# jdhuang-csm/bayes-drt

Hardware: AMD Instinct MI355X
Metric: HMC log-posterior+grad evals/sec (81 freq x 161 tau-basis) (higher is better)
Workload: dtype f64

## Files before the change

### bayes_drt_amd/csrc/bdrt_tile_s1.h

```cpp
#pragma once
#include "bdrt_device.h"
#include <type_traits>

namespace bdrt {

static __device__ long long *g_tile_trace = nullptr;

__device__ __forceinline__ int swz(int row, int col) { return row * NC + (col ^ (row & 15)); }

template <int LPC>
__device__ __forceinline__ double hsum(double x)
{
    x = sum32(x);
    if (LPC == 64) x += __shfl_xor(x, 32);
    return x;
}

__device__ __forceinline__ void wave_sync()
{
    __builtin_amdgcn_fence(__ATOMIC_RELEASE, "wavefront");
    __builtin_amdgcn_wave_barrier();
    __builtin_amdgcn_fence(__ATOMIC_ACQUIRE, "wavefront");
}

// ... 17 lines not shown
#pragma unroll
    for (int e = 0; e < 2; ++e) {
        bX[e] = Bs + kq * NC + (col ^ (8 * e + kq));
        bY[e] = Bs + (kq + 4) * NC + (col ^ (8 * e + kq + 4));
    }
    auto load = [&](dv2 (&buf)[GPF]) {
        gp2 p = base + ((size_t)(wave + l_ti * NWV) * pairs + (size_t)l_ch * GPF) * 64;
#pragma unroll
        for (int i = 0; i < GPF; ++i) buf[i] = p[(size_t)i * 64];
        if (++l_ch == nchunk) { l_ch = 0; ++l_ti; }
    };
    auto step = [&](const dv2 (&cur)[GPF], dv2 (&nxt)[GPF], bool prefetch) {
        const int p0 = c_ch * GPF;
        const bool odd = p0 & 1;
        const double *x0 = (odd ? bX[1] : bX[0]) + p0 * (8 * NC), *x1 = (odd ? bX[0] : bX[1]) + p0 * (8 * NC);
        const double *y0 = (odd ? bY[1] : bY[0]) + p0 * (8 * NC), *y1 = (odd ? bY[0] : bY[1]) + p0 * (8 * NC);
        double bx[GPF], by[GPF];
#pragma unroll
        for (int i = 0; i < GPF; ++i) {
            bx[i] = ((i & 1) ? x1 : x0)[i * (8 * NC)];
            by[i] = ((i & 1) ? y1 : y0)[i * (8 * NC)];
        }
        __builtin_amdgcn_sched_barrier(0);
        acc0 = mfma_f64(cur[0].x, bx[0], acc0);
        acc1 = mfma_f64(cur[0].y, by[0], acc1);
        __builtin_amdgcn_sched_barrier(0);
        if (prefetch) load(nxt);
        __builtin_amdgcn_sched_barrier(0);
#pragma unroll
        for (int i = 1; i < GPF; ++i) {
            acc0 = mfma_f64(cur[i].x, bx[i], acc0);
            acc1 = mfma_f64(cur[i].y, by[i], acc1);
        }
        __builtin_amdgcn_sched_barrier(0);
        if (++c_ch == nchunk) {
            const int t = wave + c_ti * NWV;
#pragma unroll
            for (int rr = 0; rr < 4; ++rr) { const int row = 16 * t + kq + 4 * rr; Os[swz(row, col)] = acc0[rr] + acc1[rr]; }
            acc0 = d4{0.0, 0.0, 0.0, 0.0}; acc1 = d4{0.0, 0.0, 0.0, 0.0};
            c_ch = 0; ++c_ti;
        }
    };
    dv2 a[GPF], b[GPF];
    if (items > 0) load(a);
    for (int it = 0; it < items; it += 2) {
        step(a, b, it + 1 < items);
        if (it + 1 < items) step(b, a, it + 2 < items);
    }
    if (rem > 0) {
        for (int ti = 0; ti < nt; ++ti) {
            const int t = wave + ti * NWV;
            d4 r0a = {0.0, 0.0, 0.0, 0.0}, r1a = {0.0, 0.0, 0.0, 0.0};
            for (int p = nchunk * GPF; p < pairs; ++p) {
                const dv2 v = base[((size_t)t * pairs + p) * 64];
                const int r0 = 8 * p + kq, r1 = r0 + 4;
                r0a = mfma_f64(v.x, Bs[swz(r0, col)], r0a);
                r1a = mfma_f64(v.y, Bs[swz(r1, col)], r1a);
            }
#pragma unroll
            for (int rr = 0; rr < 4; ++rr) {
                const int row = 16 * t + kq + 4 * rr;
                const double prev = nchunk > 0 ? Os[swz(row, col)] : 0.0;
                Os[swz(row, col)] = prev + r0a[rr] + r1a[rr];
            }
        }
    }
}

constexpr int RW = 32 * UK + 2 * MAXBW;
constexpr int NTAP = 2 * MAXBW + 1;
constexpr int WIN = UK + NTAP - 1;

__host__ __device__ inline int s1_ku(int K) { return K <= 64 ? 2 : (K <= 96 ? 3 : (K <= 128 ? 4 : 6)); }
__host__ __device__ inline int s1_nj(int D) { return D <= 32 * 4 ? 4 : (D <= 32 * 6 ? 6 : (D <= 32 * 7 ? 7 : (D <= 32 * 11 ? 11 : 16))); }
__host__ __device__ inline int s1_zrows(const DevProblem &P) { return P.toepA == 2 ? P.zrows : 16 * P.blk[0].tilesA; }
template <int TA> __device__ __forceinline__ constexpr int toep_pad() { return TA == 2 ? 16 : 8; }
template <int TA> __device__ __forceinline__ int toep_im_row(int nf) { return TA == 2 ? (nf + 3) & ~3 : nf; }

__device__ __forceinline__ const double *s1_toep_table(const DevProblem &P, const double *smem)
{
    return smem + (size_t)NC * (P.XR + s1_zrows(P)) + (size_t)2 * NC * RW;
}

#ifndef BDRT_TOEP_STAMP
#define BDRT_TOEP_STAMP(slot)
#endif
template <bool FWD>
__device__ __forceinline__ void toep_gemm(int nf, int K, int tlen, const double *Tt, const double *Bs, double *Os, int wave, int lane)
{
    typedef const __attribute__((address_space(3))) double *lds_cptr;
    const int i = lane & 15, kq = lane >> 4, col = i;
    wave = __builtin_amdgcn_readfirstlane(wave);
    constexpr int TPP = 5;
    const int r4 = nf & 3;
    const int T = FWD ? 2 * TPP : (K >> 4);
    const int base = T & ~7, R = T - base;
    const int nqt = FWD ? (K >> 4) : 2 * TPP;
    const bool halves = R > 0 && R <= 4 && nqt % 10 == 0;
    const int npiece = base + (halves ? 2 * R : R);
    if (wave >= npiece) return;
    BDRT_TOEP_STAMP(0);

    const lds_cptr aL = (lds_cptr)(Tt + (FWD ? i - kq - 76 : kq - i));
    lds_cptr bL0 = (lds_cptr)(Bs + swz(kq, col)), bL1 = (lds_cptr)(Bs + swz(4 + kq, col)), bL2 = (lds_cptr)(Bs + swz(8 + kq, col)),
             bL3 = (lds_cptr)(Bs + swz(12 + kq, col));
    const int dI0 = FWD ? 0 : swz(nf + kq, col) - swz(kq, col), dI1 = FWD ? 0 : swz(nf + 4 + kq, col) - swz(4 + kq, col),
              dI2 = FWD ? 0 : swz(nf + 8 + kq, col) - swz(8 + kq, col), dI3 = FWD ? 0 : swz(nf + 12 + kq, col) - swz(12 + kq, col);
    const int mpart = kq >= r4 ? 1 : 0, mn = nf - r4 + kq - mpart * r4;
    const lds_cptr mL = (lds_cptr)(Tt + mpart * tlen + 8 + mn - i + (K - 1));
    double Bm = 0.0;
    if (!FWD && r4) Bm = Bs[swz(kq < 2 * r4 ? mpart * nf + mn : 2 * nf + kq, col)];

    int t = 0, half = -1, orow = 0, nblk = 0, nrem = 0, aoff = 0, boff = 0;
    bool mixed = false;
    lds_cptr a, b0, b1, b2, b3;
    double A0[4], B0[4], A1[4], B1[4], A2[4], B2[4], Am = 0.0;
    d4 acc0 = {0.0, 0.0, 0.0, 0.0}, acc1 = {0.0, 0.0, 0.0, 0.0};

    auto describe = [&](int sidx) {
        t = sidx; half = -1;
        if (sidx >= base && halves) { t = base + ((sidx - base) >> 1); half = (sidx - base) & 1; }
        if (FWD) {
            const int part = t >= TPP ? 1 : 0, n0 = 16 * (t - part * TPP);
            orow = part * nf + n0;
            const int nch = (K + 3) >> 2, nq = nch >> 2;
            const int q0 = half == 1 ? nq / 2 : 0, q1 = half == 0 ? nq / 2 : nq;
            nblk = (q1 - q0) / 5; nrem = half == 0 ? 0 : nch & 3;
            aoff = part * tlen + 8 + n0 + (K - 1) - 16 * q0;
            boff = 16 * NC * q0;
            mixed = false;
        } else {
            orow = 16 * t;
            nblk = half < 0 ? 2 : 1; nrem = 0;
            aoff = 8 - 16 * t + (K - 1); boff = 0;
            mixed = r4 != 0 && half != 0;
        }
    };
    auto set_ptrs = [&](int blk) {
        if (FWD) {
            a = aL + (aoff - 80 * blk);
            const int o = boff + 80 * NC * blk;
            b0 = bL0 + o; b1 = bL1 + o; b2 = bL2 + o; b3 = bL3 + o;
        } else {
            const bool im = half == 1 || blk == 1;
            a = aL + (aoff + (im ? tlen : 0));
            b0 = bL0 + (im ? dI0 : 0); b1 = bL1 + (im ? dI1 : 0); b2 = bL2 + (im ? dI2 : 0); b3 = bL3 + (im ? dI3 : 0);
        }
    };
    auto ld = [&](double (&A)[4], double (&B)[4], auto Rr) {
        constexpr int r = decltype(Rr)::value;
#pragma unroll
        for (int j = 0; j < 4; ++j) A[j] = FWD ? a[76 - 16 * r - 4 * j] : a[16 * r + 4 * j];
        B[0] = b0[16 * NC * r]; B[1] = b1[16 * NC * r]; B[2] = b2[16 * NC * r]; B[3] = b3[16 * NC * r];
    };
    typedef std::integral_constant<int, 0> R0;
    typedef std::integral_constant<int, 1> R1;
    typedef std::integral_constant<int, 2> R2;
    typedef std::integral_constant<int, 3> R3;
    typedef std::integral_constant<int, 4> R4;
    auto mm = [&](const double (&A)[4], const double (&B)[4], auto &&next) {
        acc0 = mfma_f64(A[0], B[0], acc0);
        __builtin_amdgcn_sched_barrier(0);
        next();
        __builtin_amdgcn_sched_barrier(0);
        acc1 = mfma_f64(A[1], B[1], acc1);
        acc0 = mfma_f64(A[2], B[2], acc0);
        acc1 = mfma_f64(A[3], B[3], acc1);
        __builtin_amdgcn_sched_barrier(0);
    };
    auto block = [&](auto &&after) {
        mm(A2, B2, [&]() { ld(A0, B0, R1()); });
        mm(A0, B0, [&]() { ld(A1, B1, R2()); });
        mm(A1, B1, [&]() { ld(A0, B0, R3()); });
        mm(A0, B0, [&]() { ld(A1, B1, R4()); });
        mm(A1, B1, after);
    };
    auto open = [&](int sidx) {
        describe(sidx);
        set_ptrs(0);
        ld(A2, B2, R0());
        if (!FWD && mixed) Am = mL[-16 * t];
    };

    open(wave);
    BDRT_TOEP_STAMP(1);
    for (int sidx = wave; sidx < npiece; sidx += 8) {
        const bool more = sidx + 8 < npiece;
        const int o_row = orow, o_half = half, o_nrem = nrem;
        const bool o_mixed = mixed;
        const double o_Am = Am;
        const int nb = nblk;
        for (int blk = 0; blk < nb; ++blk) {
            const bool last = blk + 1 == nb;
            block([&]() {
                if (!last) { set_ptrs(blk + 1); ld(A2, B2, R0()); }
                else if (FWD && o_nrem) { set_ptrs(nb); ld(A2, B2, R0()); }
                else if (more) open(sidx + 8);
            });
        }
        if (FWD && o_nrem) {
            double ra[3] = {A2[0], A2[1], A2[2]}, rb[3] = {B2[0], B2[1], B2[2]};
            acc0 = mfma_f64(ra[0], rb[0], acc0);
            if (o_nrem > 1) acc1 = mfma_f64(ra[1], rb[1], acc1);
            if (o_nrem > 2) acc0 = mfma_f64(ra[2], rb[2], acc0);
            __builtin_amdgcn_sched_barrier(0);
            if (more) open(sidx + 8);
        }
        if (!FWD && o_mixed) acc1 = mfma_f64(o_Am, Bm, acc1);
        __builtin_amdgcn_sched_barrier(0);
        BDRT_TOEP_STAMP(2 + 3 * (sidx >> 3));
        const d4 s = acc0 + acc1;
        BDRT_TOEP_STAMP(3 + 3 * (sidx >> 3));
#pragma unroll
        for (int rr = 0; rr < 4; ++rr) {
            double *o = Os + swz(o_row + kq + 4 * rr, col);
            if (o_half < 0) *o = s[rr];
            else __hip_atomic_fetch_add(o, s[rr], __ATOMIC_RELAXED, __HIP_MEMORY_SCOPE_WORKGROUP);
        }
        acc0 = d4{0.0, 0.0, 0.0, 0.0}; acc1 = d4{0.0, 0.0, 0.0, 0.0};
        BDRT_TOEP_STAMP(4 + 3 * (sidx >> 3));
    }
}

template <bool FWD>
__device__ __forceinline__ void toep_zero_split(int nf, int K, double *Os, int tid)
{
    const int TPP = nf >> 4, T = FWD ? 2 * TPP : (K >> 4);
    const int base = T & ~7, R = T - base;
    if (R == 0 || R > 4 || (FWD ? (K >> 4) : 2 * TPP) % 10 != 0) return;
    for (int e = tid; e < R * 256; e += NT) {
        const int t = base + (e >> 8), r = (e >> 4) & 15;
        const int part = (FWD && t >= TPP) ? 1 : 0;
        const int row = FWD ? part * nf + 16 * (t - part * TPP) + r : 16 * t + r;
        Os[row * NC + (e & 15)] = 0.0;
    }
}

struct ToepSched { int base, R, mode, npiece; };
__host__ __device__ inline ToepSched toep_sched(int T, bool can_halve)
{
    ToepSched sc;
    sc.base = T & ~7; sc.R = T - sc.base;
    sc.mode = (sc.R == 0 || !can_halve || sc.R == 7) ? 0 : (sc.R <= 4 ? 1 : 2);
    sc.npiece = sc.base + (sc.mode == 0 ? sc.R : (sc.mode == 1 ? 2 * sc.R : 2 * sc.R - 4));
    return sc;
}
__host__ __device__ inline int toep_gen_tiles(int m) { return (m & 15) <= 2 ? (m >> 4) : ((m + 15) >> 4); }
__host__ __device__ inline int toep_gen_odd(int m) { return (m & 15) <= 2 ? (m & 15) : 0; }

constexpr int TOEP_STEPS = 8;
constexpr int TOEP_STEP_WORDS = 2 * 8 * TOEP_STEPS * 2;
inline int toep_gen_steps(bool fwd, int nf, int K, int tlen, int wave, unsigned *out)
{
    const int PAD = 16;
    const int nfi = (nf + 3) & ~3;
    const int TPP = fwd ? toep_gen_tiles(nf) : 0;
    const int T = fwd ? 2 * TPP : toep_gen_tiles(K);
    const int nch = fwd ? (K + 3) >> 2 : nfi >> 2;
    const int nq = nch >> 2;
    const int qsplit = (nq + 1) >> 1;
    const int lim = fwd ? nf : K;
    if (nq < 2 || nq > 12) return -1;
    const ToepSched sc = toep_sched(T, fwd ? nq >= 4 : true);
    int n = 0;
    bool shared_seen = false;
    auto emit = [&](int part, int n0, int q0, int kind, int shared) {
        const int aoff = fwd ? part * tlen + PAD + n0 + (K - 1) - 16 * q0 : part * tlen + PAD - n0 + (K - 1);
        const int orow = fwd ? part * nfi + n0 : n0;
        int room = lim - n0; room = room > 16 ? 16 : room;
        if (aoff < 0 || aoff > 65535 || q0 > 255 || orow > 4095 || n >= TOEP_STEPS - 1) return -1;
        out[2 * n] = (unsigned)aoff | (unsigned)q0 << 16 | (unsigned)kind << 24 | (unsigned)(fwd ? 0 : part) << 30;
        out[2 * n + 1] = (unsigned)orow | (unsigned)room << 12 | (unsigned)shared << 21 | 1u << 24;
        ++n;
        return 0;
    };
    for (int s = wave; s < sc.npiece; s += 8) {
        int t = s, half = -1;
        if (s >= sc.base) {
            const int j = s - sc.base;
            if (sc.mode == 1) { t = sc.base + (j >> 1); half = j & 1; }
            else if (sc.mode == 2 && j >= 4) { t = sc.base + 4 + ((j - 4) >> 1); half = (j - 4) & 1; }
        }
        if (shared_seen) return -1;
        if (half >= 0) shared_seen = true;
        if (fwd) {
            const int part = t >= TPP ? 1 : 0, n0 = 16 * (t - part * TPP);
            if (emit(part, n0, half == 1 ? qsplit : 0, half + 1, half >= 0 ? 1 : 0)) return -1;
        } else if (half < 0) {
            if (emit(0, 16 * t, 0, 0, 0) || emit(1, 16 * t, 0, 0, 0)) return -1;
        } else if (emit(half, 16 * t, 0, 0, 1)) return -1;
    }
    const int runs = n;
    if (runs == 0) { out[0] = (unsigned)(PAD + K - 1); out[1] = 0; }
    else { out[2 * n] = out[0]; out[2 * n + 1] = out[1] & ~(1u << 24); }
    ++n;
    for (; n < TOEP_STEPS; ++n) { out[2 * n] = out[2 * runs]; out[2 * n + 1] = out[2 * runs + 1]; }
    return runs;
}

template <int I, int N, class F>
__device__ __forceinline__ void toep_static_for(F &&f)
{
// ... 89 lines not shown
    if (!((c1 >> 24) & 1u)) return;
    prefetch(c0);
    auto body = [&](auto Lc) {
        constexpr int L = decltype(Lc)::value;
        int st = 1;
        if (FWD) {
            while (((c1 >> 24) & 1u) && ((c0 >> 24) & 3u) == 0) {
                const unsigned n0w = __builtin_amdgcn_readlane(w0v, st), n1w = __builtin_amdgcn_readlane(w1v, st);
                ++st;
                run(Lc, Tr(), n0w, nr);
                store(c1);
                c0 = n0w; c1 = n1w;
            }
            if ((c1 >> 24) & 1u) {
                const unsigned n0w = __builtin_amdgcn_readlane(w0v, st);
                if (((c0 >> 24) & 3u) == 1) run(std::integral_constant<int, (L + 1) / 2 >= 2 ? (L + 1) / 2 : 2>(), Tr(), n0w, 0);
                else run(std::integral_constant<int, L / 2 >= 2 ? L / 2 : 2>(), Tr(), n0w, nr);
                store(c1);
            }
        } else {
            while (((c1 >> 24) & 1u) && !((c1 >> 21) & 1u)) {
                const unsigned m0w = __builtin_amdgcn_readlane(w0v, st);
                const unsigned n0w = __builtin_amdgcn_readlane(w0v, st + 1), n1w = __builtin_amdgcn_readlane(w1v, st + 1);
                st += 2;
                run(Lc, Tr(), m0w, nr);
                run(Lc, Fa(), n0w, nr);
                store(c1);
                c0 = n0w; c1 = n1w;
            }
            if ((c1 >> 24) & 1u) {
                const unsigned n0w = __builtin_amdgcn_readlane(w0v, st);
                run(Lc, Tr(), n0w, nr);
                store(c1);
            }
        }
    };
    switch (nq) {
    case 2: body(std::integral_constant<int, 2>()); break;
    case 3: body(std::integral_constant<int, 3>()); break;
    case 4: body(std::integral_constant<int, 4>()); break;
    case 5: body(std::integral_constant<int, 5>()); break;
    case 6: body(std::integral_constant<int, 6>()); break;
    case 7: body(std::integral_constant<int, 7>()); break;
    case 8: body(std::integral_constant<int, 8>()); break;
    case 9: if constexpr (FWD) body(std::integral_constant<int, 9>()); break;
    case 10: if constexpr (FWD) body(std::integral_constant<int, 10>()); break;
    case 11: if constexpr (FWD) body(std::integral_constant<int, 11>()); break;
    case 12: if constexpr (FWD) body(std::integral_constant<int, 12>()); break;
    default: break;
    }
}

template <bool FWD>
__device__ __forceinline__ void toep_zero_split_gen(int nf, int K, double *Os, int tid)
{
    const int nfi = (nf + 3) & ~3;
    const int TPP = FWD ? toep_gen_tiles(nf) : 0;
    const int T = FWD ? 2 * TPP : toep_gen_tiles(K);
    const ToepSched sc = toep_sched(T, FWD ? (((K + 3) >> 2) >> 2) >= 4 : true);
    if (sc.mode == 0) return;
    const int first = sc.mode == 1 ? sc.base : sc.base + 4, cnt = sc.mode == 1 ? sc.R : sc.R - 4;
    for (int e = tid; e < cnt * 256; e += NT) {
        const int t = first + (e >> 8), r = (e >> 4) & 15;
        const int part = (FWD && t >= TPP) ? 1 : 0;
        const int n = FWD ? 16 * (t - part * TPP) + r : 16 * t + r;
        if (n < (FWD ? nf : K)) Os[(FWD ? part * nfi + n : n) * NC + (e & 15)] = 0.0;
    }
}

__device__ __forceinline__ void s1_toep_init(const DevProblem &P, double *smem)
{
    const DevBlock &B = P.blk[0];
    double *Tt = const_cast<double *>(s1_toep_table(P, smem));
    double *Zh = smem + (size_t)P.XR * NC;
    const int glen = P.nf + B.K - 1, tlen = P.tlen, pad = P.toepA == 2 ? 16 : 8;
    for (int e = threadIdx.x; e < 2 * tlen; e += NT) {
        const int part = e >= tlen ? 1 : 0, j = e - part * tlen - pad;
        Tt[e] = (j >= 0 && j < glen) ? B.tg[(size_t)part * glen + j] : 0.0;
    }
    if (P.toepA == 2) {
        unsigned *st = (unsigned *)(Tt + 2 * tlen);
        for (int e = threadIdx.x; e < TOEP_STEP_WORDS; e += NT) st[e] = P.tsteps[e];
    }
    for (int e = (P.toepA == 2 ? 0 : 2 * P.nf * NC) + threadIdx.x; e < s1_zrows(P) * NC; e += NT) Zh[e] = 0.0;
    __syncthreads();
}

__device__ __forceinline__ double *s1_grad_row(const DevProblem &P, double *smem, int c);


__host__ __device__ inline size_t s1_lds_doubles(const DevProblem &P)
{
    return (size_t)NC * (P.XR + s1_zrows(P)) + (size_t)2 * NC * RW + (P.toepA ? (size_t)2 * P.tlen : 0) + (P.toepA == 2 ? (size_t)TOEP_STEP_WORDS / 2 : 0);
}

struct NoHook { __device__ __forceinline__ void operator()() const {} };

template <bool LDSIO, int LPC = 32, class Hook = NoHook, class Hook1 = NoHook, int TA = 0, int KU = 6>
__device__ inline void logp_grad_tile_s1(const DevProblem &P, const TileIO &io, double *smem, Hook before_backward = Hook(),
                                         Hook1 after_x_ready = Hook1())
{
    int tid = threadIdx.x;
    __asm__ volatile("" : "+v"(tid));
    constexpr int UKV = 32 * KU / LPC, UNV = 128 / LPC, WINV = UKV + NTAP - 1, NWV = 16 * LPC / 64;
    constexpr int GPFV = LPC == 32 ? 7 : 3;
    const int lane = tid & 63, wave = tid >> 6;
    const int c = tid / LPC;
    const int l32 = tid % LPC, hb = lane & (64 - LPC);
    const DevBlock &B = P.blk[0];
    const int nf = P.nf, N2 = 2 * nf, K = B.K, KP = 8 * B.kpairs;
    const int omode = LDSIO ? 0 : P.outlier_mode;
    const int dbg = P.dbg;
    const bool valid = c < io.nvalid;
    const int cc = valid ? c : 0;
    const double jac = io.jacobian ? 1.0 : 0.0;

    double *Xs = smem;
    double *Zh = Xs + (size_t)P.XR * NC;
    double *xrow = Zh + (size_t)(TA == 2 ? P.zrows : 16 * B.tilesA) * NC + (size_t)c * (2 * RW);
    double *wrow = xrow + RW;

    const double *th = io.theta + (long)cc * io.t_sc;
    typedef const __attribute__((address_space(3))) double *lds_cptr;
    auto TH = [&](int j) -> double { return LDSIO ? ((lds_cptr)th)[j] : th[(long)j * io.t_sj]; };
    double *gr = (io.grad && valid) ? io.grad + (long)cc * io.g_sc : nullptr;
    auto GW = [&](int j, double v) { if (!LDSIO && gr) gr[(long)j * io.g_sj] = v; };
    double gsc = 0.0;
    double *pr = (!LDSIO && io.params && valid) ? io.params + (size_t)cc * P.D : nullptr;
    auto PW = [&](int j, double v) { if (!LDSIO && pr) pr[j] = v; };

    long long tprev = (io.prof && tid == 0) ? clock64() : 0;
    long long *trc = g_tile_trace ? g_tile_trace + ((size_t)blockIdx.x * NWV + wave) * 16 : nullptr;
#define BDRT_S1_TRACE(slot) do { if (trc && (lane == 0)) trc[slot] = clock64(); } while (0)
    BDRT_S1_TRACE(0);
#define BDRT_S1_PROF(slot) do { if (io.prof && tid == 0) { const long long t_ = clock64(); io.prof[slot] += t_ - tprev; tprev = t_; } } while (0)
    long long twe = io.prof ? clock64() : 0;
#define BDRT_S1_BARRIER(slot, wslot) do { if (io.prof) { const long long tb_ = clock64(); __syncthreads(); const long long te_ = clock64(); \
        if (lane == 0) { atomicAdd((unsigned long long *)&io.prof[slot], (unsigned long long)(te_ - tb_)); \
                         if (wslot) atomicAdd((unsigned long long *)&io.prof[wslot], (unsigned long long)(tb_ - twe)); } \
        twe = te_; } else __syncthreads(); } while (0)

    double sraw = 0.0, st = 0.0;
    {
        int j = -1;
        if (l32 < 2) j = l32;
        else if (l32 < 6) j = P.o_err + (l32 - 2);
        else if (l32 < 9) j = B.o_d + (l32 - 6);
        if (j >= 0) { st = TH(j); sraw = lean_exp(st); PW(j, sraw); }
    }
    double lp = 0.0;
    int lp_lane = -1;
    double x_[UKV];
    {
        double tx_[UKV], tu_[UKV];
#pragma unroll
        for (int u = 0; u < UKV; ++u) {
            const int k = l32 + LPC * u, kk = k < K ? k : 0;
            tx_[u] = TH(B.o_x + kk);
            tu_[u] = TH(B.o_ups + kk);
        }
#pragma unroll
        for (int u = 0; u < UKV; ++u) {
            const bool in = l32 + LPC * u < K;
            tx_[u] = in ? tx_[u] : 0.0;
            tu_[u] = in ? tu_[u] : 0.0;
        }
        double ex_[UKV];
#pragma unroll
        for (int u = 0; u < UKV; ++u) ex_[u] = lean_exp(tx_[u]);
#pragma unroll
        for (int u = 0; u < UKV; ++u) {
            const int k = l32 + LPC * u;
            double xr = 0.0;
            if (k < K) {
                xr = B.is_pos ? ex_[u] : tx_[u];
                if (B.is_pos) lp += jac * tx_[u];
                PW(B.o_x + k, xr);
            }
            x_[u] = xr;
            if (k < KP) Xs[swz(k, c)] = xr;
            xrow[MAXBW + k] = xr;
            wrow[MAXBW + k] = tu_[u];
        }
        if (l32 < MAXBW) {
            xrow[l32] = 0.0; xrow[MAXBW + LPC * UKV + l32] = 0.0;
            wrow[l32] = 0.0; wrow[MAXBW + LPC * UKV + l32] = 0.0;
        }
    }
    static_assert(!TA || LPC == 32, "the Toeplitz-A GEMMs are written for 512 threads");
    const double *Tt = TA ? s1_toep_table(P, smem) : nullptr;
    const int tlen = TA ? P.tlen : 0;
    constexpr int TPAD = toep_pad<TA>();
    const int nfi = toep_im_row<TA>(nf);
    if (TA) {
        const int r16 = TA == 2 ? toep_gen_odd(nf) : (nf & 15), n0 = nf - r16;
        for (int j = 0; j < r16; ++j) {
            double sr = 0.0, si = 0.0;
#pragma unroll
            for (int u = 0; u < UKV; ++u) {
                const int idx = max(TPAD + n0 + j + (K - 1) - (l32 + LPC * u), 0);
                sr = fma(Tt[idx], x_[u], sr); si = fma(Tt[tlen + idx], x_[u], si);
            }
            sr = hsum<LPC>(sr); si = hsum<LPC>(si);
            if (l32 == 0) { Zh[swz(n0 + j, c)] = sr; Zh[swz(nfi + n0 + j, c)] = si; }
        }
        if (TA == 2) toep_zero_split_gen<true>(nf, K, Zh, tid); else toep_zero_split<true>(nf, K, Zh, tid);
    }
    const double d0 = __shfl(sraw, hb | 6), d1 = __shfl(sraw, hb | 7), d2 = __shfl(sraw, hb | 8);
    const double israw5 = 5.0 * lean_rcp(sraw);
    if (l32 < 6) lp += -0.5 * sraw * sraw + jac * st;
    else if (l32 < 9) lp += -6.0 * st - israw5 + jac * st;
#ifndef BDRT_SPEC_EARLY
#define BDRT_SPEC_EARLY 0
#endif
#ifndef BDRT_EARLY_P2
#define BDRT_EARLY_P2 1
#endif
#ifndef BDRT_P2_OPAQUE_K
#define BDRT_P2_OPAQUE_K 1
#endif
    constexpr bool EARLY_P2 = BDRT_EARLY_P2 != 0;
    double zre_[UNV], zim_[UNV], wn_[UNV];
    auto load_spectrum = [&]() {
        const int sp = io.spec ? io.spec[cc] : 0;
        const double *Zm = P.Z + (size_t)sp * N2;
#pragma unroll
        for (int v = 0; v < UNV; ++v) {
            const int n = l32 + LPC * v, nn = n < nf ? n : 0;
            zre_[v] = Zm[nn]; zim_[v] = Zm[nf + nn]; wn_[v] = P.w[nn];
        }
    };
#pragma unroll 1
    for (int step = 0; step < 2; ++step) {
    if (EARLY_P2 ? step == 1 : step == 0) {
        BDRT_S1_TRACE(1);
        BDRT_S1_BARRIER(25, 29);
        after_x_ready();
        if constexpr (BDRT_SPEC_EARLY) load_spectrum();
        BDRT_S1_TRACE(2);
        BDRT_S1_PROF(1);
        BDRT_S1_TRACE(3);
        if (!(dbg & 1)) {
            if (TA == 2) toep_gemm_gen<true>(nf, K, tlen, Tt, Xs, Zh, wave, lane);
            else if (TA) toep_gemm<true>(nf, K, tlen, Tt, Xs, Zh, wave, lane);
            else gemm_sw<NWV, GPFV>(B.Af, B.tilesA, B.kpairs, Xs, Zh, wave, lane);
        }
        continue;
    }

    BDRT_S1_TRACE(4);
    if (!(dbg & 4)) {
        const int kb = UKV * l32;
        double xw[WINV], tuc[UKV];
#pragma unroll
        for (int j = 0; j < WINV; ++j) xw[j] = xrow[kb + j];
#pragma unroll
        for (int u = 0; u < UKV; ++u) tuc[u] = wrow[MAXBW + kb + u];
        wave_sync();
        double v0_[UKV], v1_[UKV], v2_[UKV];
#pragma unroll
        for (int u = 0; u < UKV; ++u) { v0_[u] = 0.0; v1_[u] = 0.0; v2_[u] = 0.0; }
        double tn0 = B.T[0][0], tn1 = B.T[1][0], tn2 = B.T[2][0];
#pragma unroll
        for (int d = 0; d < NTAP; ++d) {
            const double t0 = tn0, t1 = tn1, t2 = tn2;
            if (d + 1 < NTAP) { tn0 = B.T[0][d + 1]; tn1 = B.T[1][d + 1]; tn2 = B.T[2][d + 1]; }
            __asm__ volatile("" ::: "memory");
#pragma unroll
            for (int u = 0; u < UKV; ++u) { v0_[u] = fma(t0, xw[u + d], v0_[u]); v1_[u] = fma(t1, xw[u + d], v1_[u]); v2_[u] = fma(t2, xw[u + d], v2_[u]); }
        }
        double ue[UKV + 4], ie[UKV + 2];
#pragma unroll
        for (int u = 0; u < UKV; ++u) { ue[u + 2] = 0.15 * lean_exp(tuc[u]); ie[u + 1] = lean_rcp(ue[u + 2]); }
        {
            const int lo = hb | ((l32 + LPC - 1) & (LPC - 1)), hi = hb | ((l32 + 1) & (LPC - 1));
            ue[0] = __shfl(ue[UKV], lo); ue[1] = __shfl(ue[UKV + 1], lo);
            ue[UKV + 2] = __shfl(ue[2], hi); ue[UKV + 3] = __shfl(ue[3], hi);
            ie[0] = __shfl(ie[UKV], lo); ie[UKV + 1] = __shfl(ie[1], hi);
        }
        BDRT_S1_PROF(5);
        double sv0 = 0, sv1 = 0, sv2 = 0;
        double w0_[UKV], w1_[UKV], w2_[UKV], gup[UKV];
#pragma unroll
        for (int u = 0; u < UKV; ++u) {
            int k = kb + u;
#if BDRT_P2_OPAQUE_K
            __asm__ volatile("" : "+v"(k));
#endif
            w0_[u] = 0.0; w1_[u] = 0.0; w2_[u] = 0.0; gup[u] = 0.0;
            if (k < K) {
                const double um2 = ue[u], um1 = ue[u + 1], uu = ue[u + 2], up1 = ue[u + 3], up2 = ue[u + 4];
                const double t = tuc[u];
                const double iu = ie[u + 1], iu2 = iu * iu;
                const double v0 = v0_[u], v1 = v1_[u], v2 = v2_[u];
                const double q2 = d0 * v0 * v0 + d1 * v1 * v1 + d2 * v2 * v2;
                const double ir = 0.15 * iu;
                lp += -(t + LOG_015) - 0.5 * q2 * iu2 - (P.ups_alpha + 1.0) * t - P.ups_beta * ir + jac * t;
                sv0 += v0 * v0 * iu2; sv1 += v1 * v1 * iu2; sv2 += v2 * v2 * iu2;
                double gu = -iu + q2 * iu2 * iu;
                if (k >= 1 && k + 1 < K) {
                    const double du = 0.5 * (uu - 0.5 * (um1 + up1)) * iu;
                    lp += -0.5 * du * du;
                    gu += -du * 0.25 * (um1 + up1) * iu2;
                }
                if (k >= 2) {
                    const double i0 = ie[u];
                    const double du = 0.5 * (um1 - 0.5 * (um2 + uu)) * i0;
                    gu += du * 0.25 * i0;
                }
                if (k + 2 < K) {
                    const double i0 = ie[u + 2];
                    const double du = 0.5 * (up1 - 0.5 * (uu + up2)) * i0;
                    gu += du * 0.25 * i0;
                }
                gup[u] = uu * gu - (P.ups_alpha + 1.0) + P.ups_beta * ir + jac;
                PW(B.o_ups + k, uu * (1.0 / 0.15));
                w0_[u] = -d0 * v0 * iu2; w1_[u] = -d1 * v1 * iu2; w2_[u] = -d2 * v2 * iu2;
            }
            __builtin_amdgcn_sched_barrier(0);
        }
        double gl_[UKV];
#pragma unroll
        for (int u = 0; u < UKV; ++u) gl_[u] = 0.0;
#pragma unroll
        for (int i = 0; i < 3; ++i) {
#pragma unroll
            for (int u = 0; u < UKV; ++u) wrow[MAXBW + kb + u] = i == 0 ? w0_[u] : (i == 1 ? w1_[u] : w2_[u]);
// ... 60 lines not shown
        for (int v = 0; v < UNV; ++v) {
            const int n = l32 + LPC * v;
            if (n >= nf) continue;
            const double wn = wn_[v];
            const double zr = azr_[v] + Rinf;
            const double zi = azi_[v] + induc * wn;
            double so_re = 0.0, so_im = 0.0, r0 = 0.0, r1 = 0.0, t0 = 0.0, t1 = 0.0;
            if (omode) {
                t0 = TH(P.o_so + n); t1 = TH(P.o_so + nf + n);
                r0 = lean_exp(t0); r1 = lean_exp(t1);
                PW(P.o_so + n, r0); PW(P.o_so + nf + n, r1);
                if (omode == 1) so_re = so_im = 0.05 * r0 * r1;
                else { so_re = 0.05 * r0; so_im = 0.05 * r1; }
            }
            const double common = ar2 * zr * zr + ai2 * zi * zi;
            const double s2_re = c0 + ap2 * zr * zr + common + so_re * so_re;
            const double s2_im = c0 + ap2 * zi * zi + common + so_im * so_im;
            const double e_re = zre_[v] - zr, e_im = zim_[v] - zi;
            const double prod = s2_re * s2_im, ip = lean_rcp(prod);
            const double w_re = s2_im * ip, w_im = s2_re * ip;
            if (v < UNV / 2) pp_lo *= prod; else pp_hi *= prod;
            lp += -0.5 * e_re * e_re * w_re - 0.5 * e_im * e_im * w_im;
            const double h_re = -0.5 * w_re + 0.5 * e_re * e_re * w_re * w_re;
            const double h_im = -0.5 * w_im + 0.5 * e_im * e_im * w_im * w_im;
            const double gzr = e_re * w_re + 2.0 * zr * (h_re * (ap2 + ar2) + h_im * ar2);
            const double gzi = e_im * w_im + 2.0 * zi * (h_im * (ap2 + ai2) + h_re * ai2);
            Zh[swz(n, c)] = gzr;
            Zh[swz(nfi + n, c)] = gzi;
            if (TA && rk > 0) {
                lk0 = fma(tk0r_[v], gzr, fma(tk0i_[v], gzi, lk0));
                if (rk > 1) lk1 = fma(tk1r_[v], gzr, fma(tk1i_[v], gzi, lk1));
            }
            sR += gzr;
            sL += gzi * wn;
            sH += h_re + h_im;
            sHz2 += h_re * zr * zr + h_im * zi * zi;
            sHzr2 += (h_re + h_im) * zr * zr;
            sHzi2 += (h_re + h_im) * zi * zi;
            if (omode == 1) {
                const double dso = 2.0 * so_re * (h_re + h_im);
                GW(P.o_so + n, r0 * (0.05 * r1 * dso - P.so_lambda) + jac);
                GW(P.o_so + nf + n, 0.05 * r0 * r1 * dso - (P.so_alpha + 1.0) + P.so_beta / r1 + jac);
                lp += -P.so_lambda * r0 - (P.so_alpha + 1.0) * t1 - P.so_beta / r1 + jac * (t0 + t1);
            } else if (omode == 2) {
                GW(P.o_so + n, r0 * (0.05 * 2.0 * so_re * h_re - P.so_lambda) + jac);
                GW(P.o_so + nf + n, r1 * (0.05 * 2.0 * so_im * h_im - P.so_lambda) + jac);
                lp += -P.so_lambda * (r0 + r1) + jac * (t0 + t1);
            }
            if (!LDSIO && io.Z_hat && valid) { io.Z_hat[(size_t)c * N2 + n] = zr; io.Z_hat[(size_t)c * N2 + nf + n] = zi; }
            if (!LDSIO && io.sigma_tot && valid) {
                io.sigma_tot[(size_t)c * N2 + n] = sqrt(s2_re);
                io.sigma_tot[(size_t)c * N2 + nf + n] = sqrt(s2_im);
            }
        }
        lp += -0.5 * lean_log(pp_lo);
        if (nf > LPC * (UNV / 2)) lp += -0.5 * lean_log(pp_hi);
        double dl = 0.0;
        if constexpr (LPC == 32) {
            const double q[8] = {sR, sL, sH, sHz2, sHzr2, sHzi2, lk0, lp};
            const double tot = sum32_by_lane<8>(q, l32);
            dl = (l32 == 0 ? 100.0 : (l32 == 1 ? P.induc_scale : 0.005 * sraw)) * tot;
            if (TA && rk > 0) {
                if (l32 == 6) Xs[swz(K - rk, c)] = tot;
                if (rk > 1) { lk1 = hsum<LPC>(lk1); if (l32 == 0) Xs[swz(K - rk + 1, c)] = lk1; }
            }
            lp = tot;
            lp_lane = 7;
        } else {
            sR = hsum<LPC>(sR); sL = hsum<LPC>(sL); sH = hsum<LPC>(sH); sHz2 = hsum<LPC>(sHz2); sHzr2 = hsum<LPC>(sHzr2); sHzi2 = hsum<LPC>(sHzi2);
            if (l32 == 0) dl = 100.0 * sR;
            else if (l32 == 1) dl = P.induc_scale * sL;
            else if (l32 == 2) dl = 0.05 * 2.0 * s_res * sH;
            else if (l32 == 3) dl = 0.05 * 2.0 * a_p * sHz2;
            else if (l32 == 4) dl = 0.05 * 2.0 * a_r * sHzr2;
            else dl = 0.05 * 2.0 * a_i * sHzi2;
        }
        if (l32 < 6) {
            const int j = l32 < 2 ? l32 : P.o_err + (l32 - 2);
            gsc = sraw * (dl - sraw) + jac;
            GW(j, gsc);
        }
    }
    BDRT_S1_TRACE(7);
    BDRT_S1_BARRIER(27, 31);
    BDRT_S1_TRACE(8);
    BDRT_S1_PROF(4);
    before_backward();
    if (!(dbg & 2)) {
        if (TA == 2) toep_gemm_gen<false>(nf, K, tlen, Tt, Zh, Xs, wave, lane);
        else if (TA) toep_gemm<false>(nf, K, tlen, Tt, Zh, Xs, wave, lane);
        else gemm_sw<NWV, GPFV>(B.BkA, B.tilesK, B.rpairsA, Zh, Xs, wave, lane);
    }
    BDRT_S1_TRACE(9);
    BDRT_S1_BARRIER(28, 0);
    BDRT_S1_TRACE(10);
    BDRT_S1_PROF(8);

    double gx_[UKV], gu_[UKV];
    {
        double ag_[UKV], gl2_[UKV];
#pragma unroll
        for (int u = 0; u < UKV; ++u) {
            const int k = l32 + LPC * u, kk = k < K ? k : 0;
            ag_[u] = Xs[swz(kk, c)]; gl2_[u] = wrow[MAXBW + k]; gu_[u] = xrow[MAXBW + k];
        }
#pragma unroll
        for (int u = 0; u < UKV; ++u) {
            const int k = l32 + LPC * u;
            const double graw = ag_[u] + gl2_[u];
            const double gx = B.is_pos ? x_[u] * graw + jac : graw;
            gx_[u] = k < K ? gx : 0.0;
            gu_[u] = k < K ? gu_[u] : 0.0;
            if (!LDSIO && k < K) { GW(B.o_x + k, gx_[u]); GW(B.o_ups + k, gu_[u]); }
        }
    }
    if (LDSIO) {
        wave_sync();
#pragma unroll
        for (int u = 0; u < UKV; ++u) {
            const int k = l32 + LPC * u;
            if (k < K) { xrow[B.o_x + k] = gx_[u]; xrow[B.o_ups + k] = gu_[u]; }
        }
        if (l32 < 9) xrow[l32 < 2 ? l32 : (l32 < 6 ? P.o_err + (l32 - 2) : B.o_d + (l32 - 6))] = gsc;
    }
    if (lp_lane < 0) { lp = hsum<LPC>(lp); lp_lane = 0; }
    if (l32 == lp_lane && io.lp && valid) io.lp[c] = lp;
    BDRT_S1_PROF(9);
    BDRT_S1_TRACE(11);
    if (LDSIO) wave_sync(); else __syncthreads();
}

__device__ __forceinline__ double *s1_grad_row(const DevProblem &P, double *smem, int c)
{
    return smem + (size_t)NC * (P.XR + s1_zrows(P)) + (size_t)c * (2 * RW);
}

}
```

Baseline: 170.0 million.

## Precompute per-lane Toeplitz GEMM LDS addresses in a shared table and prefetch before barrier

Builds a per-lane LDS table holding the swizzled byte addresses for the X, Z, imaginary-Z, Toeplitz and mixed-row operands once at setup. Each wave loads these addresses with vector LDS reads before the barrier, so they are no longer recomputed inside toep_gemm. The gemm loop itself is restructured: pointer and next-piece description work is moved into the MFMA pipeline, the remainder operands are loaded early, and the first MFMA takes zero as input so the accumulators need no explicit reset. This cuts integer address arithmetic and VGPR pressure on the critical path, at the cost of extra LDS space and table reads.

```diff
diff --git a/bayes_drt_amd/csrc/bdrt_tile_s1.h b/bayes_drt_amd/csrc/bdrt_tile_s1.h
--- a/bayes_drt_amd/csrc/bdrt_tile_s1.h
+++ b/bayes_drt_amd/csrc/bdrt_tile_s1.h
@@ -123,16 +123,74 @@
     return smem + (size_t)NC * (P.XR + s1_zrows(P)) + (size_t)2 * NC * RW;
 }
 
+constexpr int TOEP_LANE_DOUBLES = 64 * 16 / 2 + 2;
+constexpr int TOEP_FWD_BIAS = 92;
+typedef unsigned toep_u4 __attribute__((ext_vector_type(4)));
+
+__device__ __forceinline__ unsigned toep_lds_addr(const void *p)
+{
+    return (unsigned)(size_t)(const __attribute__((address_space(3))) char *)p;
+}
+__device__ __forceinline__ unsigned toep_lane_table(const double *Tt, int tlen) { return (toep_lds_addr(Tt + 2 * tlen) + 15u) & ~15u; }
+
+__device__ __forceinline__ void toep_lane_table_fill(int nf, int K, int tlen, const double *Tt, const double *Xs, const double *Zh, int tid)
+{
+    if (tid >= 64) return;
+    typedef __attribute__((address_space(3))) toep_u4 *lds_q;
+    const lds_q Lt = (lds_q)(size_t)toep_lane_table(Tt, tlen);
+    const int i = tid & 15, kq = tid >> 4, col = i;
+    const int r4 = nf & 3;
+    toep_u4 x, z, d, m;
+#pragma unroll
+    for (int j = 0; j < 4; ++j) {
+        x[j] = toep_lds_addr(Xs + swz(4 * j + kq, col));
+        z[j] = toep_lds_addr(Zh + swz(4 * j + kq, col));
+        d[j] = toep_lds_addr(Zh + swz(nf + 4 * j + kq, col));
+    }
+    const int mpart = kq >= r4 ? 1 : 0, mn = nf - r4 + kq - mpart * r4;
+    m[0] = toep_lds_addr(Tt + (i - kq - TOEP_FWD_BIAS));
+    m[1] = toep_lds_addr(Tt + (kq - i));
+    m[2] = toep_lds_addr(Tt + (mpart * tlen + 8 + mn - i + (K - 1)));
+    m[3] = toep_lds_addr(Zh + swz(kq < 2 * r4 ? mpart * nf + mn : 2 * nf + kq, col));
+    Lt[tid] = x; Lt[64 + tid] = z; Lt[128 + tid] = d; Lt[192 + tid] = m;
+}
+
+#ifndef BDRT_TOEP_OPAQUE
+#define BDRT_TOEP_OPAQUE 1
+#endif
+struct ToepLane { toep_u4 qM, qX, qZ; };
+template <bool FWD>
+__device__ __forceinline__ ToepLane toep_lane_fetch(int K, int tlen, const double *Tt, int wave, int lane)
+{
+    typedef const __attribute__((address_space(3))) toep_u4 *lds_q;
+    wave = __builtin_amdgcn_readfirstlane(wave);
+    const unsigned lrow = toep_lane_table(Tt, tlen) + 16u * (unsigned)lane;
+    ToepLane L;
+    L.qM = *(lds_q)(size_t)(lrow + 3072);
+    L.qX = *(lds_q)(size_t)(lrow);
+    if (!FWD) {
+        const int T = K >> 4, base = T & ~7, R = T - base;
+        const int im0 = (wave >= base && R > 0 && R <= 4) ? (wave - base) & 1 : 0;
+        L.qZ = *(lds_q)(size_t)(lrow + 1024u + 1024u * (unsigned)im0);
+    } else L.qZ = L.qX;
+    return L;
+}
+
 #ifndef BDRT_TOEP_STAMP
 #define BDRT_TOEP_STAMP(slot)
 #endif
 template <bool FWD>
-__device__ __forceinline__ void toep_gemm(int nf, int K, int tlen, const double *Tt, const double *Bs, double *Os, int wave, int lane)
+__device__ __forceinline__ void toep_gemm(int nf, int K, int tlen, const double *Tt, int wave, int lane, const ToepLane &pre)
 {
     typedef const __attribute__((address_space(3))) double *lds_cptr;
-    const int i = lane & 15, kq = lane >> 4, col = i;
+    typedef __attribute__((address_space(3))) double *lds_ptr;
+    typedef const __attribute__((address_space(3))) toep_u4 *lds_q;
     wave = __builtin_amdgcn_readfirstlane(wave);
+#if BDRT_TOEP_OPAQUE
+    __asm__ volatile("" : "+s"(K));
+#endif
     constexpr int TPP = 5;
+    constexpr int DB = (int)sizeof(double);
     const int r4 = nf & 3;
     const int T = FWD ? 2 * TPP : (K >> 4);
     const int base = T & ~7, R = T - base;
@@ -142,123 +200,128 @@
     if (wave >= npiece) return;
     BDRT_TOEP_STAMP(0);
 
-    const lds_cptr aL = (lds_cptr)(Tt + (FWD ? i - kq - 76 : kq - i));
-    lds_cptr bL0 = (lds_cptr)(Bs + swz(kq, col)), bL1 = (lds_cptr)(Bs + swz(4 + kq, col)), bL2 = (lds_cptr)(Bs + swz(8 + kq, col)),
-             bL3 = (lds_cptr)(Bs + swz(12 + kq, col));
-    const int dI0 = FWD ? 0 : swz(nf + kq, col) - swz(kq, col), dI1 = FWD ? 0 : swz(nf + 4 + kq, col) - swz(4 + kq, col),
-              dI2 = FWD ? 0 : swz(nf + 8 + kq, col) - swz(8 + kq, col), dI3 = FWD ? 0 : swz(nf + 12 + kq, col) - swz(12 + kq, col);
-    const int mpart = kq >= r4 ? 1 : 0, mn = nf - r4 + kq - mpart * r4;
-    const lds_cptr mL = (lds_cptr)(Tt + mpart * tlen + 8 + mn - i + (K - 1));
+    const unsigned lrow = toep_lane_table(Tt, tlen) + 16u * (unsigned)lane;
+    auto LQ = [&](int quad) -> toep_u4 { return *(lds_q)(size_t)(lrow + (unsigned)(1024 * quad)); };
+    const toep_u4 qM = pre.qM, qX = pre.qX;
+    const unsigned aL = FWD ? qM[0] : qM[1];
     double Bm = 0.0;
-    if (!FWD && r4) Bm = Bs[swz(kq < 2 * r4 ? mpart * nf + mn : 2 * nf + kq, col)];
-
-    int t = 0, half = -1, orow = 0, nblk = 0, nrem = 0, aoff = 0, boff = 0;
+    if (!FWD && r4) Bm = *(lds_cptr)(size_t)qM[3];
+
+    int half = -1, nblk = 0, nrem = 0, aoff = 0, boff = 0, ooff = 0, im = 0, nxt = 0;
     bool mixed = false;
-    lds_cptr a, b0, b1, b2, b3;
-    double A0[4], B0[4], A1[4], B1[4], A2[4], B2[4], Am = 0.0;
-    d4 acc0 = {0.0, 0.0, 0.0, 0.0}, acc1 = {0.0, 0.0, 0.0, 0.0};
+    unsigned a, b0, b1, b2, b3, am = 0;
+    toep_u4 qZ, qOut;
+    double A0[4], B0[4], A1[4], B1[4], A2[4], B2[4], Ar[3], Br[3], Am = 0.0;
+    d4 acc0, acc1;
 
     auto describe = [&](int sidx) {
-        t = sidx; half = -1;
+        int t = sidx; half = -1;
         if (sidx >= base && halves) { t = base + ((sidx - base) >> 1); half = (sidx - base) & 1; }
         if (FWD) {
-            const int part = t >= TPP ? 1 : 0, n0 = 16 * (t - part * TPP);
-            orow = part * nf + n0;
+            const int part = 1 - (int)((unsigned)(t - TPP) >> 31), n0 = 16 * (t - part * TPP);
             const int nch = (K + 3) >> 2, nq = nch >> 2;
             const int q0 = half == 1 ? nq / 2 : 0, q1 = half == 0 ? nq / 2 : nq;
             nblk = (q1 - q0) / 5; nrem = half == 0 ? 0 : nch & 3;
-            aoff = part * tlen + 8 + n0 + (K - 1) - 16 * q0;
-            boff = 16 * NC * q0;
+            aoff = DB * (part * tlen + 8 + n0 + (K - 1) - 16 * q0);
+            boff = DB * 16 * NC * q0;
+            ooff = DB * NC * n0; im = part;
             mixed = false;
         } else {
-            orow = 16 * t;
             nblk = half < 0 ? 2 : 1; nrem = 0;
-            aoff = 8 - 16 * t + (K - 1); boff = 0;
+            aoff = DB * (8 - 16 * t + (K - 1)); boff = 0;
+            ooff = DB * NC * 16 * t; im = (half + 1) >> 1;
             mixed = r4 != 0 && half != 0;
         }
     };
-    auto set_ptrs = [&](int blk) {
-        if (FWD) {
-            a = aL + (aoff - 80 * blk);
-            const int o = boff + 80 * NC * blk;
-            b0 = bL0 + o; b1 = bL1 + o; b2 = bL2 + o; b3 = bL3 + o;
-        } else {
-            const bool im = half == 1 || blk == 1;
-            a = aL + (aoff + (im ? tlen : 0));
-            b0 = bL0 + (im ? dI0 : 0); b1 = bL1 + (im ? dI1 : 0); b2 = bL2 + (im ? dI2 : 0); b3 = bL3 + (im ? dI3 : 0);
-        }
-    };
+    auto LD = [](unsigned p, int off) -> double { return *(lds_cptr)(size_t)(p + (unsigned)(DB * off)); };
     auto ld = [&](double (&A)[4], double (&B)[4], auto Rr) {
         constexpr int r = decltype(Rr)::value;
 #pragma unroll
-        for (int j = 0; j < 4; ++j) A[j] = FWD ? a[76 - 16 * r - 4 * j] : a[16 * r + 4 * j];
-        B[0] = b0[16 * NC * r]; B[1] = b1[16 * NC * r]; B[2] = b2[16 * NC * r]; B[3] = b3[16 * NC * r];
+        for (int j = 0; j < 4; ++j) A[j] = FWD ? LD(a, TOEP_FWD_BIAS - 16 * r - 4 * j) : LD(a, 16 * r + 4 * j);
+        B[0] = LD(b0, 16 * NC * r); B[1] = LD(b1, 16 * NC * r); B[2] = LD(b2, 16 * NC * r); B[3] = LD(b3, 16 * NC * r);
     };
     typedef std::integral_constant<int, 0> R0;
     typedef std::integral_constant<int, 1> R1;
     typedef std::integral_constant<int, 2> R2;
     typedef std::integral_constant<int, 3> R3;
     typedef std::integral_constant<int, 4> R4;
-    auto mm = [&](const double (&A)[4], const double (&B)[4], auto &&next) {
-        acc0 = mfma_f64(A[0], B[0], acc0);
+    typedef std::integral_constant<bool, true> First;
+    typedef std::integral_constant<bool, false> Later;
+    auto fetch_ptrs = [&](int blk) { nxt = blk; if (!FWD) qZ = LQ(1 + (im | blk)); };
+    auto request = [&]() {
+        if (FWD) {
+            a = aL + (unsigned)(aoff - DB * 80 * nxt);
+            const unsigned o = (unsigned)(boff + DB * 80 * NC * nxt);
+            b0 = qX[0] + o; b1 = qX[1] + o; b2 = qX[2] + o; b3 = qX[3] + o;
+        } else {
+            a = aL + (unsigned)(aoff + (im | nxt) * (DB * tlen));
+            b0 = qZ[0]; b1 = qZ[1]; b2 = qZ[2]; b3 = qZ[3];
+            am = qM[2] - (unsigned)ooff / NC;
+        }
+        ld(A2, B2, R0());
+    };
+    auto prepare = [&](auto first, int blk, int nb, int sidx) {
+        if (FWD) {
+#pragma unroll
+            for (int j = 0; j < 3; ++j) Ar[j] = LD(a, TOEP_FWD_BIAS - 80 - 4 * j);
+            Br[0] = LD(b0, 80 * NC); Br[1] = LD(b1, 80 * NC); Br[2] = LD(b2, 80 * NC);
+            if constexpr (decltype(first)::value) qOut = LQ(1 + im);
+        } else Am = LD(am, 0);
+        const bool last = blk + 1 >= nb;
+        if (last) describe(sidx + 8 < npiece ? sidx + 8 : sidx);
+        fetch_ptrs(last ? 0 : blk + 1);
+    };
+    auto mm = [&](const double (&A)[4], const double (&B)[4], auto first, auto &&next) {
+        constexpr bool zero = decltype(first)::value;
+        const d4 z = {0.0, 0.0, 0.0, 0.0};
+        if constexpr (zero) acc0 = mfma_f64(A[0], B[0], z); else acc0 = mfma_f64(A[0], B[0], acc0);
         __builtin_amdgcn_sched_barrier(0);
         next();
         __builtin_amdgcn_sched_barrier(0);
-        acc1 = mfma_f64(A[1], B[1], acc1);
+        if constexpr (zero) acc1 = mfma_f64(A[1], B[1], z); else acc1 = mfma_f64(A[1], B[1], acc1);
         acc0 = mfma_f64(A[2], B[2], acc0);
         acc1 = mfma_f64(A[3], B[3], acc1);
         __builtin_amdgcn_sched_barrier(0);
     };
-    auto block = [&](auto &&after) {
-        mm(A2, B2, [&]() { ld(A0, B0, R1()); });
-        mm(A0, B0, [&]() { ld(A1, B1, R2()); });
-        mm(A1, B1, [&]() { ld(A0, B0, R3()); });
-        mm(A0, B0, [&]() { ld(A1, B1, R4()); });
-        mm(A1, B1, after);
-    };
-    auto open = [&](int sidx) {
-        describe(sidx);
-        set_ptrs(0);
-        ld(A2, B2, R0());
-        if (!FWD && mixed) Am = mL[-16 * t];
-    };
-
-    open(wave);
+    auto block = [&](auto first, auto &&prep) {
+        mm(A2, B2, first, [&]() { ld(A0, B0, R1()); });
+        mm(A0, B0, Later(), [&]() { ld(A1, B1, R2()); });
+        mm(A1, B1, Later(), [&]() { ld(A0, B0, R3()); });
+        mm(A0, B0, Later(), [&]() { ld(A1, B1, R4()); prep(); });
+        mm(A1, B1, Later(), request);
+    };
+
+    describe(wave);
+    nxt = 0; qZ = pre.qZ;
+    request();
     BDRT_TOEP_STAMP(1);
     for (int sidx = wave; sidx < npiece; sidx += 8) {
-        const bool more = sidx + 8 < npiece;
-        const int o_row = orow, o_half = half, o_nrem = nrem;
+        const int o_off = ooff, o_half = half, o_nrem = nrem;
         const bool o_mixed = mixed;
-        const double o_Am = Am;
         const int nb = nblk;
-        for (int blk = 0; blk < nb; ++blk) {
-            const bool last = blk + 1 == nb;
-            block([&]() {
-                if (!last) { set_ptrs(blk + 1); ld(A2, B2, R0()); }
-                else if (FWD && o_nrem) { set_ptrs(nb); ld(A2, B2, R0()); }
-                else if (more) open(sidx + 8);
-            });
-        }
+        block(First(), [&]() { prepare(First(), 0, nb, sidx); });
+        for (int blk = 1; blk < nb; ++blk) block(Later(), [&]() { prepare(Later(), blk, nb, sidx); });
         if (FWD && o_nrem) {
-            double ra[3] = {A2[0], A2[1], A2[2]}, rb[3] = {B2[0], B2[1], B2[2]};
-            acc0 = mfma_f64(ra[0], rb[0], acc0);
-            if (o_nrem > 1) acc1 = mfma_f64(ra[1], rb[1], acc1);
-            if (o_nrem > 2) acc0 = mfma_f64(ra[2], rb[2], acc0);
-            __builtin_amdgcn_sched_barrier(0);
-            if (more) open(sidx + 8);
-        }
-        if (!FWD && o_mixed) acc1 = mfma_f64(o_Am, Bm, acc1);
+            acc0 = mfma_f64(Ar[0], Br[0], acc0);
+            if (o_nrem > 1) acc1 = mfma_f64(Ar[1], Br[1], acc1);
+            if (o_nrem > 2) acc0 = mfma_f64(Ar[2], Br[2], acc0);
+        }
+        if (!FWD && o_mixed) acc1 = mfma_f64(Am, Bm, acc1);
         __builtin_amdgcn_sched_barrier(0);
         BDRT_TOEP_STAMP(2 + 3 * (sidx >> 3));
         const d4 s = acc0 + acc1;
         BDRT_TOEP_STAMP(3 + 3 * (sidx >> 3));
-#pragma unroll
-        for (int rr = 0; rr < 4; ++rr) {
-            double *o = Os + swz(o_row + kq + 4 * rr, col);
-            if (o_half < 0) *o = s[rr];
-            else __hip_atomic_fetch_add(o, s[rr], __ATOMIC_RELAXED, __HIP_MEMORY_SCOPE_WORKGROUP);
-        }
-        acc0 = d4{0.0, 0.0, 0.0, 0.0}; acc1 = d4{0.0, 0.0, 0.0, 0.0};
+        unsigned o[4];
+#pragma unroll
+        for (int rr = 0; rr < 4; ++rr) { o[rr] = (FWD ? qOut[rr] : qX[rr]) + (unsigned)o_off; __asm__ volatile("" : "+v"(o[rr])); }
+        if (o_half < 0) {
+#pragma unroll
+            for (int rr = 0; rr < 4; ++rr) *(lds_ptr)(size_t)o[rr] = s[rr];
+        } else {
+#pragma unroll
+            for (int rr = 0; rr < 4; ++rr)
+                __hip_atomic_fetch_add((lds_ptr)(size_t)o[rr], s[rr], __ATOMIC_RELAXED, __HIP_MEMORY_SCOPE_WORKGROUP);
+        }
         BDRT_TOEP_STAMP(4 + 3 * (sidx >> 3));
     }
 }
@@ -514,6 +577,7 @@
         unsigned *st = (unsigned *)(Tt + 2 * tlen);
         for (int e = threadIdx.x; e < TOEP_STEP_WORDS; e += NT) st[e] = P.tsteps[e];
     }
+    if (P.toepA == 1) toep_lane_table_fill(P.nf, B.K, tlen, Tt, smem, Zh, threadIdx.x);
     for (int e = (P.toepA == 2 ? 0 : 2 * P.nf * NC) + threadIdx.x; e < s1_zrows(P) * NC; e += NT) Zh[e] = 0.0;
     __syncthreads();
 }
@@ -523,7 +587,8 @@
 
 __host__ __device__ inline size_t s1_lds_doubles(const DevProblem &P)
 {
-    return (size_t)NC * (P.XR + s1_zrows(P)) + (size_t)2 * NC * RW + (P.toepA ? (size_t)2 * P.tlen : 0) + (P.toepA == 2 ? (size_t)TOEP_STEP_WORDS / 2 : 0);
+    return (size_t)NC * (P.XR + s1_zrows(P)) + (size_t)2 * NC * RW + (P.toepA ? (size_t)2 * P.tlen : 0) + (P.toepA == 1 ? (size_t)TOEP_LANE_DOUBLES : 0) +
+           (P.toepA == 2 ? (size_t)TOEP_STEP_WORDS / 2 : 0);
 }
 
 struct NoHook { __device__ __forceinline__ void operator()() const {} };
@@ -648,6 +713,9 @@
 #ifndef BDRT_EARLY_P2
 #define BDRT_EARLY_P2 1
 #endif
+#ifndef BDRT_TOEP_PREFETCH
+#define BDRT_TOEP_PREFETCH 1
+#endif
 #ifndef BDRT_P2_OPAQUE_K
 #define BDRT_P2_OPAQUE_K 1
 #endif
@@ -666,6 +734,8 @@
     for (int step = 0; step < 2; ++step) {
     if (EARLY_P2 ? step == 1 : step == 0) {
         BDRT_S1_TRACE(1);
+        ToepLane tlane;
+        if (TA == 1 && BDRT_TOEP_PREFETCH) tlane = toep_lane_fetch<true>(K, tlen, Tt, wave, lane);
         BDRT_S1_BARRIER(25, 29);
         after_x_ready();
         if constexpr (BDRT_SPEC_EARLY) load_spectrum();
@@ -674,7 +744,10 @@
         BDRT_S1_TRACE(3);
         if (!(dbg & 1)) {
             if (TA == 2) toep_gemm_gen<true>(nf, K, tlen, Tt, Xs, Zh, wave, lane);
-            else if (TA) toep_gemm<true>(nf, K, tlen, Tt, Xs, Zh, wave, lane);
+            else if (TA) {
+                if (!BDRT_TOEP_PREFETCH) tlane = toep_lane_fetch<true>(K, tlen, Tt, wave, lane);
+                toep_gemm<true>(nf, K, tlen, Tt, wave, lane, tlane);
+            }
             else gemm_sw<NWV, GPFV>(B.Af, B.tilesA, B.kpairs, Xs, Zh, wave, lane);
         }
         continue;
@@ -901,13 +974,18 @@
         }
     }
     BDRT_S1_TRACE(7);
+    ToepLane tlane;
+    if (TA == 1 && BDRT_TOEP_PREFETCH) tlane = toep_lane_fetch<false>(K, tlen, Tt, wave, lane);
     BDRT_S1_BARRIER(27, 31);
     BDRT_S1_TRACE(8);
     BDRT_S1_PROF(4);
     before_backward();
     if (!(dbg & 2)) {
         if (TA == 2) toep_gemm_gen<false>(nf, K, tlen, Tt, Zh, Xs, wave, lane);
-        else if (TA) toep_gemm<false>(nf, K, tlen, Tt, Zh, Xs, wave, lane);
+        else if (TA) {
+            if (!BDRT_TOEP_PREFETCH) tlane = toep_lane_fetch<false>(K, tlen, Tt, wave, lane);
+            toep_gemm<false>(nf, K, tlen, Tt, wave, lane, tlane);
+        }
         else gemm_sw<NWV, GPFV>(B.BkA, B.tilesK, B.rpairsA, Zh, Xs, wave, lane);
     }
     BDRT_S1_TRACE(9);
```

After: 174.7 million, median of 6. 1.03x the previous value.
